# LTLA/batchelor

Measured on AMD Instinct MI355X. Metric: cells/sec corrected (reducedMNN engine, 50 PCs), higher is better.
Workload: dtype fp16 MFMA candidate pass (f32 accumulate) + FP64 exact re-rank; 1 GPU; config3: 8 synthetic Gaussian batches x 100000 cells x 50 PCs, k=20, merge.order=1..8, inputs resident in HBM; parallelism=single GPU, exact_fallback_queries=1050

## Files before the change

batchelor_amd/_lib.py:

```python
from __future__ import annotations

import ctypes
import os

import numpy as np

_HERE = os.path.dirname(os.path.abspath(__file__))
LIB_PATH = os.environ.get("BMX_LIB") or os.path.join(_HERE, "libbatchelor_mi355x.so")

c_i32p = ctypes.POINTER(ctypes.c_int32)
c_i64p = ctypes.POINTER(ctypes.c_int64)
c_f64p = ctypes.POINTER(ctypes.c_double)

_lib = None


class BatchelorMI355XError(RuntimeError):
    def __init__(self, code, message):
        super().__init__(message)
        self.code = code


def lib():
    global _lib
    if _lib is None:
        if not os.path.exists(LIB_PATH):
            raise ImportError(
                f"{LIB_PATH} is missing: build it with `python -c 'import __graft_entry__ as g; g.build()'` "
                "(or `make -C batchelor_amd/csrc`). There is no CPU fallback for the MI355X hot path.")
        try:
            import torch
        except Exception:
            pass
        _lib = ctypes.CDLL(LIB_PATH, mode=ctypes.RTLD_GLOBAL)
        _lib.bmx_last_error.restype = ctypes.c_char_p
        _lib.bmx_device_count.restype = ctypes.c_int32
        _lib.bmx_last_knn_exact_fallbacks.restype = ctypes.c_int64
        _lib.bmx_free.argtypes = [ctypes.c_void_p]
        _lib.bmx_free.restype = None
    return _lib


def check(rc):
    if rc != 0:
        raise BatchelorMI355XError(rc, lib().bmx_last_error().decode("utf-8", "replace"))


def dev_set(name, value):
    check(lib().bmx_dev_set(name.encode(), ctypes.c_int32(int(value))))


def dev_get(name):
    v = ctypes.c_int64(0)
    check(lib().bmx_dev_get(name.encode(), ctypes.byref(v)))
    return int(v.value)


def dev_get_bytes(name, n):
    out = np.zeros(int(n), dtype=np.uint8)
    check(lib().bmx_dev_get_bytes(name.encode(), out.ctypes.data_as(ctypes.c_void_p), ctypes.c_int64(int(n))))
    return out


def device_count():
    return int(lib().bmx_device_count())


def require_gpu():
    if device_count() < 1:
        raise BatchelorMI355XError(-1, "no MI355X / HIP device visible: the batchelor_amd hot path has no CPU fallback")


def f64p(a):
    return a.ctypes.data_as(c_f64p)


def i32p(a):
    return a.ctypes.data_as(c_i32p)


def as_f(a):
    return np.asfortranarray(a, dtype=np.float64)


# ... 8 lines not shown
```

batchelor_amd/csrc/abi.hip:

```cpp
#include <algorithm>
#include <chrono>
#include <climits>
#include <cstddef>
#include <cmath>
#include <cstdlib>
#include <cstring>
#include <functional>
#include <limits>
#include <memory>
#include <thread>
#include <vector>

#include "bmx_common.hpp"
#include "bmx_ops.hpp"
#include "engine.hpp"
#include "host_xfer.hpp"
#include "mnn_correct.hpp"
#include "rccl_dyn.hpp"
#include "resident_batches.hpp"

struct bmx_engine {
    std::unique_ptr<bmx::Engine> impl;
};
struct bmx_mnn_result {
    int B = 0;
    bmx::MnnCorrectResult r;
};

namespace {

thread_local std::string g_last_error;
thread_local int64_t g_last_fallbacks = 0;
thread_local int g_force_exact = 0;
thread_local std::unique_ptr<bmx::Engine> g_prim;

bmx::Engine& prim(int d) {
    if (!g_prim) {
        int dev = 0;
        BMX_HIP(hipGetDevice(&dev));
        g_prim = std::make_unique<bmx::Engine>(dev);
    }
    g_prim->d_ = d;
    g_prim->knn_ws_.force_exact = g_force_exact;
    return *g_prim;
}

template <class T>
T* upload(bmx::DevBuf<T>& buf, const T* host, size_t n, hipStream_t s) {
    T* p = buf.reserve(std::max<size_t>(n, 1));
// ... 115 lines not shown
        }
    });
}

void bmx_trim_caches(void) {
    bmx::DevBlockCache::release_global();
    bmx::StreamPool::release_all();
}

int64_t bmx_last_knn_exact_fallbacks(void) { return g_last_fallbacks; }

void bmx_set_force_exact_knn(int32_t on) { g_force_exact = on; }

int32_t bmx_dev_set(const char* name, int32_t value) {
    if (!name) return BMX_ERR_ARG;
    bmx::DevKnobs& k = bmx::dev_knobs();
    const std::string n(name);
    if (n == "knn_tier") k.knn_tier = value;
    else if (n == "sample") k.sample = value;
    else if (n == "split_c") k.split_c = value;
    else if (n == "force_c") k.force_c = value;
    else if (n == "no_margin") k.no_margin = value;
    else if (n == "asv_fast") k.asv_fast = value;
    else if (n == "asv_cap") k.asv_cap = value;
    else if (n == "sample_split") k.sample_split = value;
    else if (n == "lk_seed") k.lk_seed = value;
    else if (n == "asv_modes") k.asv_modes = value;
    else if (n == "asv_sync") k.asv_sync = value;
    else if (n == "tau_replay") k.tau_replay = value;
    else if (n == "exchange_always") k.exchange_always = value;
    else if (n == "refine_wave") k.refine_wave = value;
    else if (n == "asv_wide") k.asv_wide = value;
    else if (n == "asv_chunk") k.asv_chunk = value;
    else if (n == "reset") k = bmx::DevKnobs();
    else {
        g_last_error = "bmx_dev_set: unknown knob '" + n + "'";
        return BMX_ERR_ARG;
    }
    return BMX_OK;
}

int32_t bmx_dev_get(const char* name, int64_t* value) {
    if (!name || !value) return BMX_ERR_ARG;
    return guarded([&] {
        const std::string n(name);
        unsigned long long t[8];
        if (n == "asv_literal_cells" || n == "asv_fallback_cells" || n == "asv_tiled_cells") {
            bmx::asv_tally_read(t, false);
            *value = (int64_t)t[n == "asv_literal_cells" ? 0 : (n == "asv_fallback_cells" ? 1 : 2)];
        } else if (n == "asv_ticks_stream" || n == "asv_ticks_wait" || n == "asv_ticks_cells") {
            bmx::asv_ticks_read(t);
            *value = (int64_t)t[n == "asv_ticks_stream" ? 0 : (n == "asv_ticks_wait" ? 1 : 2)];
        } else if (n == "asv_ticks_literal" || n == "asv_ticks_chains" || n == "asv_literal_addends" || n == "asv_chain_tiles") {
            bmx::asv_ticks_read(t);
            *value = (int64_t)t[n == "asv_ticks_literal" ? 4 : (n == "asv_ticks_chains" ? 5 : (n == "asv_literal_addends" ? 6 : 7))];
        } else if (n == "delta_gene_tile" || n == "delta_pair_chunk") {
            *value = n == "delta_gene_tile" ? bmx::DELTA_GENE_TILE : bmx::DELTA_PAIR_CHUNK;
        } else if (n == "pca_sparse_row_segment") {
            *value = bmx::PCA_SPARSE_ROW_SEGMENT;
        } else if (n == "asv_tally_reset") {
            bmx::asv_tally_read(t, true);
            *value = 0;
        } else {
            throw bmx::Error(BMX_ERR_ARG, "bmx_dev_get: unknown counter '" + n + "'");
        }
    });
}

int32_t bmx_dev_get_bytes(const char* name, void* dst, int64_t n) {
    if (!name || (n > 0 && !dst) || n < 0) return BMX_ERR_ARG;
    return guarded([&] {
        if (std::string(name) != "asv_modes") throw bmx::Error(BMX_ERR_ARG, std::string("bmx_dev_get_bytes: unknown array '") + name + "'");
// ... 719 lines not shown
```

batchelor_amd/csrc/bmx_common.hpp:

```cpp
#pragma once
#include <hip/hip_runtime.h>

#include <atomic>
#include <cstdint>
#include <cstdio>
#include <map>
#include <mutex>
#include <stdexcept>
#include <string>
#include <vector>

#include "../../include/batchelor_mi355x.h"

namespace bmx {

struct Error : std::runtime_error {
    int code;
    Error(int c, const std::string& m) : std::runtime_error(m), code(c) {}
};

#define BMX_HIP(expr)                                                                                   \
    do {                                                                                                \
        hipError_t e_ = (expr);                                                                         \
        if (e_ != hipSuccess)                                                                           \
            throw bmx::Error(BMX_ERR_HIP, std::string(#expr) + " failed: " + hipGetErrorString(e_));    \
    } while (0)

#define BMX_LAUNCH_CHECK() BMX_HIP(hipGetLastError())

struct WatchdogTimeout : Error {
    explicit WatchdogTimeout(const std::string& m) : Error(BMX_ERR_HIP, m) {}
};
void guarded_stream_sync(hipStream_t stream, double budget_s);

#ifndef BMX_KS1
#define BMX_KS1 32
#endif

struct DevKnobs {
    int knn_tier = 0;
    int sample = -1;
    int split_c = 0;
    int force_c = 0;
    int no_margin = 0;
    int asv_fast = 0;
    int asv_cap = -1;
    int asv_modes = 0;
    int asv_sync = 0;
    int tau_replay = 0;
    int lk_seed = 1;
    int sample_split = -1;
    int exchange_always = 0;
    int refine_wave = 0;
    int asv_wide = 0;
    int asv_chunk = 0;
};
DevKnobs& dev_knobs();
bool debug_prints();
bool debug_timings();

inline int cdiv(int64_t a, int64_t b) { return (int)((a + b - 1) / b); }
inline int64_t round_up(int64_t a, int64_t b) { return (a + b - 1) / b * b; }

struct DevBlockCache {
    struct Block {
        void* p;
        size_t bytes;
        int device;
    };
    std::vector<Block> blocks;
    bool leak = false;
    DevBlockCache() = default;
    DevBlockCache(const DevBlockCache&) = delete;
    DevBlockCache& operator=(const DevBlockCache&) = delete;
    struct GlobalPool {
        std::mutex mu;
        std::vector<Block> blocks;
        size_t total = 0;
    };
    static GlobalPool& global() {
        static GlobalPool* g = new GlobalPool();
        return *g;
    }
    ~DevBlockCache() {
        GlobalPool& g = global();
        if (!leak) {
            std::lock_guard<std::mutex> lk(g.mu);
            for (const Block& b : blocks) {
// ... 298 lines not shown
        return events[events_used++];
    }
    ~KnnWorkspace() {
        if (abandon) return;
        pinned_small_give(pin_);
        for (auto& e : events) {
            (void)hipEventDestroy(e.first);
            (void)hipEventDestroy(e.second);
        }
    }
};

struct Bf16Launch {
    const uint16_t* pq;
    const uint16_t* pr;
    int nqb, first_begin, range_len, nranges, r_limit, out_chunk0, out_nchunks;
    uint32_t* tau_g;
    int sample;
    int32_t* cand;
    float* cand_v;
    float* tau;
    int n_full = 0;
    const float* margin = nullptr;
    int k = 0;
    const uint32_t* tau_seed = nullptr;
};
int bf16_pick_ns(int d);
int bf16_ncons(int NS, int KS);
void bf16_prep(hipStream_t stream, const double* X, const int32_t* rows, int n, int n_pad, int d, int NS,
               const double* mean, int is_query, uint16_t* P, double* n2, unsigned long long* maxbits,
               unsigned long long* slots);
bool bf16_launch(hipStream_t stream, KnnWorkspace& ws, int NS, int KS, const Bf16Launch& L);
int f16_rows_per_slot(int NS, int KS);

void knn_device(hipStream_t stream, KnnWorkspace& ws, const double* X, const int32_t* ref_rows, int nr,
                const double* Q, const int32_t* q_rows, int nq, int d, int k, int32_t* idx_out, double* dist_out,
                int q_begin, int q_end, const float* seed_d2 = nullptr, const double* centre = nullptr,
                double* kth_out = nullptr);

}
```

batchelor_amd/csrc/knn.hip:

```cpp
#include "bmx_common.hpp"
#include "knn_select.hpp"

#include <algorithm>
#include <atomic>
#include <chrono>
#include <cmath>
#include <cstdio>
#include <cstdlib>
#include <thread>

namespace bmx {

int f16_pick_ns(int d, int KS);
void f16_prep_all(hipStream_t stream, const double* X, const int32_t* rrows, int nr, int nr_pad, const double* Q,
                  const int32_t* qrows, int nq, int nq_pad, int d, int NS, const double* mean, uint16_t* Pr, uint16_t* Pq,
                  double* rn2, double* qn2, unsigned long long* maxbits, unsigned long long* slots, int32_t* flagged0,
                  float* margin, const sel::PassEps& pe, const float* seed_d2, uint32_t* tau_seed, uint32_t* tau_init);
bool f16_launch(hipStream_t stream, KnnWorkspace& ws, int NS, int KS, const Bf16Launch& L);
void f16_sample_merge(hipStream_t stream, const float* lists, int nranges, int KS, int nq, int k, const float* margin,
                      uint32_t* tau_g);

namespace {

using namespace sel;

constexpr int MAX_CHUNKS = 8;

__global__ void colsum_partial(const double* __restrict__ X, const int32_t* __restrict__ rows, int n, int d,
                               int rows_per_block, int stride, double* __restrict__ partial) {
    __shared__ double sm[4][64];
    const int c0 = threadIdx.x & 63, rl = threadIdx.x >> 6;
    const int r0 = blockIdx.x * rows_per_block;
    const int r1 = min(n, r0 + rows_per_block);
    for (int cb = 0; cb < d; cb += 64) {
        const int c = cb + c0;
        double s = 0.0;
        if (c < d)
            for (int r = r0 + rl; r < r1; r += 4) {
                const int64_t rs = (int64_t)r * stride;
                const int64_t row = rows ? rows[rs] : rs;
                s += X[row * d + c];
            }
        sm[rl][c0] = s;
        __syncthreads();
        if (rl == 0 && c < d) partial[(int64_t)blockIdx.x * d + c] = (sm[0][c0] + sm[1][c0]) + (sm[2][c0] + sm[3][c0]);
        __syncthreads();
    }
}

__global__ void colsum_final(const double* __restrict__ partial, int nblocks, int d, double scale,
                             double* __restrict__ out) {
    const int c = blockIdx.x * blockDim.x + threadIdx.x;
    if (c >= d) return;
    double s = 0.0;
    for (int b = 0; b < nblocks; ++b) s += partial[(int64_t)b * d + c];
    out[c] = s * scale;
}


// ... 31 lines not shown
        const double t = a[c] - b[c];
        s += t * t;
    }
    return s;
}

__device__ __forceinline__ bool key_less(double da, int ia, double db, int ib) {
    return da < db || (da == db && ia < ib);
}

constexpr int REFINE_MAXM = MAX_CHUNKS * 48;

__global__ void seed_tau_kernel(const float* __restrict__ seed_d2, const double* __restrict__ qn2,
                                const unsigned long long* __restrict__ max_rn2_bits, int nq, int nq_pad, PassEps pe,
                                uint32_t* __restrict__ tau_g) {
    const int q = blockIdx.x * blockDim.x + threadIdx.x;
    if (q >= nq_pad) return;
    uint32_t o = f32_orderable(-__builtin_inff());
    if (q < nq) o = pass_seed_tau((double)seed_d2[q], qn2[q], __longlong_as_double((long long)*max_rn2_bits), pe);
    tau_g[q] = q < nq ? min(tau_g[q], o) : o;
}

template <int REFINE_NC>
__global__ __launch_bounds__(256) void knn_refine(const double* __restrict__ X, const int32_t* __restrict__ ref_rows,
                                                  const double* __restrict__ Q, const int32_t* __restrict__ q_rows,
                                                  int nq, int d, int k, int KS, int nchunks, double eps_k, double eps_qr,
                                                  double eps_split, double eps_den, int scaled,
                                                  const int32_t* __restrict__ cand, const float* __restrict__ cand_v,
                                                  const float* __restrict__ tau, const double* __restrict__ qn2,
                                                  const unsigned long long* __restrict__ max_rn2_bits,
                                                  const float* __restrict__ seed_d2, int32_t* __restrict__ idx_out,
                                                  double* __restrict__ dist_out, int32_t* __restrict__ flagged,
                                                  double* __restrict__ flag_bound,
                                                  unsigned long long* __restrict__ zero_slots, int q0,
                                                  double* __restrict__ kth_out, int sq = 0) {
    __shared__ __attribute__((aligned(16))) double sd[4][REFINE_MAXM];
    __shared__ int si[4][REFINE_MAXM];
    const int lane = threadIdx.x & 63, w = threadIdx.x >> 6;
    if (zero_slots && blockIdx.x == 0 && threadIdx.x < 64) zero_slots[(size_t)threadIdx.x * 16] = 0ull;
    const int q = q0 + blockIdx.x * 4 + w;
    if (q >= nq) return;
    const int Mall = nchunks * KS;
    const double* qv = Q + (int64_t)(q_rows ? q_rows[q] : q) * d;
    const double max_rn2 = __longlong_as_double((long long)*max_rn2_bits);
    const double s = scaled ? pass_scale(max_rn2) : 1.0;
    const double s2inv = 1.0 / (s * s);
    const double eps = pass_eps(sqrt(qn2[q]), sqrt(max_rn2), s, eps_k, eps_qr, eps_split, eps_den);
    int M = 0;
    unsigned long long* sk = reinterpret_cast<unsigned long long*>(&sd[w][0]);
    for (int m0 = 0; m0 < Mall; m0 += 64) {
        const int m = m0 + lane;
        const int id = m < Mall ? cand[(int64_t)q * Mall + m] : -1;
        const unsigned long long mask = __builtin_amdgcn_ballot_w64(id >= 0);
        const int pos = M + __builtin_popcountll(mask & ((1ull << lane) - 1ull));
        if (id >= 0) {
            si[w][pos] = id;
            if (cand_v) sk[pos] = ((unsigned long long)f32_orderable(cand_v[(int64_t)q * Mall + m]) << 32) | (uint32_t)id;
        }
        M += __builtin_popcountll(mask);
    }
    __builtin_amdgcn_fence(__ATOMIC_ACQ_REL, "wavefront");
    float tmerge = __builtin_inff();
    if (cand_v && M > k) {
        constexpr int NU = (REFINE_MAXM + 63) / 64;
        int rk[NU], ids[NU];
        float vs[NU];
        float vk = __builtin_inff();
#pragma unroll
        for (int uu = 0; uu < NU; ++uu) {
            const int m = lane + 64 * uu;
            rk[uu] = 0x7FFFFFFF;
            ids[uu] = 0;
            vs[uu] = 0.f;
            if (m < M) {
                const unsigned long long km = sk[m];
                const float vm = orderable_f32((uint32_t)(km >> 32));
                int rank = 0;
                int f = 0;
                for (; f + 2 <= M; f += 2) {
                    typedef unsigned long long u64x2 __attribute__((ext_vector_type(2)));
                    const u64x2 kf = *reinterpret_cast<const u64x2*>(sk + f);
                    rank += (kf[0] < km ? 1 : 0) + (kf[1] < km ? 1 : 0);
                }
                if (f < M) rank += sk[f] < km ? 1 : 0;
                rk[uu] = rank;
                ids[uu] = (int)(uint32_t)km;
                vs[uu] = vm;
                if (rank == k - 1) vk = vm;
                if (rank == KS) tmerge = vm;
            }
// ... 55 lines not shown
                        const uint32_t lo = (uint32_t)__builtin_amdgcn_update_dpp(0, (int)(uint32_t)bits, 0x93, 0xF, 0xF, false);
                        const uint32_t hi = (uint32_t)__builtin_amdgcn_update_dpp(0, (int)(uint32_t)(bits >> 32), 0x93, 0xF, 0xF, false);
                        const double prev = __longlong_as_double((long long)(((unsigned long long)hi << 32) | lo));
                        double run = prev + y[c][0];
                        run += y[c][1];
                        if (p == ph && 4 * c + ph < np) acc = run;
                    }
                }
            }
            if (p == p_last && m < M) sd[w][m] = acc;
        }
    } else {
        for (int m = lane; m < M; m += 64) {
            const int id = si[w][m];
            sd[w][m] = exact_d2(qv, X + (int64_t)(ref_rows ? ref_rows[id] : id) * d, d);
        }
    }
    __builtin_amdgcn_fence(__ATOMIC_ACQ_REL, "wavefront");
    const double seed = seed_d2 ? (double)seed_d2[q] : __builtin_inf();
    double kth = M >= k ? 0.0 : seed;
    for (int m = M + lane; m < k; m += 64) idx_out[(int64_t)q * k + m] = seed_d2 ? -1 : 0;
    for (int m = lane; m < M; m += 64) {
        const double dm = sd[w][m];
        const int im = si[w][m];
        int rank = 0;
        for (int f = 0; f < M; ++f) rank += key_less(sd[w][f], si[w][f], dm, im) ? 1 : 0;
        if (rank < k) {
            idx_out[(int64_t)q * k + rank] = im;
            if (dist_out) dist_out[(int64_t)q * k + rank] = sq ? dm : sqrt(dm);
        }
        if (rank == k - 1) kth = dm;
    }
    float tmin = tmerge;
    for (int c = lane; c < nchunks; c += 64) tmin = fminf(tmin, tau[(int64_t)q * nchunks + c]);
    for (int o = 32; o > 0; o >>= 1) {
        tmin = fminf(tmin, __shfl_xor(tmin, o));
        kth = fmax(kth, __shfl_xor(kth, o));
    }
    const double kth_full = kth;
    kth = fmin(kth, seed);
    if (lane == 0) {
        const bool proven = kth < (double)tmin * s2inv + qn2[q] - eps;
        if (!proven) {
            const int pos = atomicAdd(&flagged[0], 1);
            flagged[1 + pos] = q;
            flag_bound[pos] = kth;
        }
        if (kth_out) kth_out[q] = (proven && M >= k) ? sqrt(kth_full) : __builtin_inf();
    }
}

template <int REFINE_NC>
__global__ __launch_bounds__(256) void knn_refine_half(const double* __restrict__ X, const int32_t* __restrict__ ref_rows,
                                                       const double* __restrict__ Q, const int32_t* __restrict__ q_rows,
                                                       int nq, int d, int k, int nchunks, double eps_k, double eps_qr,
                                                       double eps_split, double eps_den, int scaled,
                                                       const int32_t* __restrict__ cand, const float* __restrict__ cand_v,
                                                       const float* __restrict__ tau, const double* __restrict__ qn2,
                                                       const unsigned long long* __restrict__ max_rn2_bits,
                                                       const float* __restrict__ seed_d2, int32_t* __restrict__ idx_out,
                                                       double* __restrict__ dist_out, int32_t* __restrict__ flagged,
                                                       double* __restrict__ flag_bound,
                                                       unsigned long long* __restrict__ zero_slots,
                                                       double* __restrict__ kth_out, int sq = 0) {
    constexpr int KS = 32;
    __shared__ __attribute__((aligned(16))) double sd[8][KS];
    __shared__ int si[8][KS];
// ... 578 lines not shown

__global__ void tau_record_kernel(const float* __restrict__ tau, int nchunks, int nq, uint32_t* __restrict__ rec) {
    const int q = blockIdx.x * blockDim.x + threadIdx.x;
    if (q >= nq) return;
    float t = __builtin_inff();
    for (int c = 0; c < nchunks; ++c) t = fminf(t, tau[(int64_t)q * nchunks + c]);
    rec[q] = f32_orderable(t);
}
__global__ void tau_apply_kernel(const uint32_t* __restrict__ rec, int nq, uint32_t* __restrict__ tau_g) {
    const int q = blockIdx.x * blockDim.x + threadIdx.x;
    if (q < nq) tau_g[q] = min(tau_g[q], rec[q]);
}

#ifndef BMX_SEEDED_SAMPLE
#define BMX_SEEDED_SAMPLE 4096
#endif
struct Tier {
    int id;
    int NS, KS;
};

int candidate_tiers(int d, int k, int nr, Tier out[2]) {
    const int only = dev_knobs().knn_tier;
    int n = 0;
    if (k > 36) return 0;
    const int KS1 = k <= 20 ? BMX_KS1 : 48, KS2 = k <= 20 ? 24 : 40;
    const int ns1 = f16_pick_ns(d, KS1);
    if (ns1 && nr > 2 * KS1 && (only == 0 || only == 1)) out[n++] = Tier{1, ns1, KS1};
    const int ns2 = bf16_pick_ns(d);
    if (ns2 && !(KS2 == 40 && ns2 > 16) && nr > 2 * KS2 && (only == 0 || only == 2)) out[n++] = Tier{2, ns2, KS2};
    return n;
}

void candidate_pass(hipStream_t stream, KnnWorkspace& ws, const Tier& T, const double* X, const int32_t* ref_rows, int nr,
                    const double* Qs, const int32_t* qrs, int nq, int d, int k, int32_t* io, double* dout,
                    int32_t* flagged, double* flag_bound, const float* seed_d2, const double* centre, double* kth_out) {
    const int NS = T.NS, KS = T.KS;
    ws.last_variant = T.id == 1 ? 3 : 2;
    const int unit = T.id == 1 ? 256 : 32 * bf16_ncons(NS, KS);
    const int nq_pad = (int)round_up(nq, unit);
    const int nqb = nq_pad / unit;

    const bool no_margin_knob = dev_knobs().no_margin != 0;
    int S_auto = nr >= 32768 ? 4096 : 0;
    if (T.id == 1 && nr >= 4096) S_auto = std::max(1024, std::min(nr / 4, NS <= 4 ? 24576 : 12288));
    if (seed_d2 && T.id == 1) S_auto = std::min(S_auto, BMX_SEEDED_SAMPLE);
    int S = (int)round_up(dev_knobs().sample >= 0 ? dev_knobs().sample : S_auto, T.id == 1 ? f16_rows_per_slot(NS, KS) : 64);
    int CS = 1;
    if (T.id == 1 && S > 0 && nqb < 128 && dev_knobs().sample_split != 0 && !no_margin_knob) {
        const int rs = f16_rows_per_slot(NS, KS);
        CS = std::max(1, std::min({256 / std::max(nqb, 1), 8, S / (8 * rs)}));
        if (dev_knobs().sample_split > 0) CS = std::max(1, std::min({dev_knobs().sample_split, S / rs, 512 / KS}));
    }
    int C = 1, n_full = 0;
    {
        const int a = nqb / 256, b = nqb % 256;
        n_full = a * 256;
        if (b > 0) {
            double best = 1e30;
            for (int c = 1; c <= MAX_CHUNKS - 1; ++c) {
                if (c > 1 && nr / c < 2048) break;
                const double tailc = std::ceil((double)b * c / 256.0) / c * (1.0 + 0.105 * std::log((double)c));
                if (tailc < best - 1e-9) {
                    best = tailc;
                    C = c;
                }
            }
        }
    }
    if (dev_knobs().split_c > 0) C = std::max(1, dev_knobs().split_c);
    if (dev_knobs().force_c > 0) {
        C = std::max(1, std::min(MAX_CHUNKS - 1, dev_knobs().force_c));
        n_full = 0;
    }
    const int rmul = T.id == 1 ? f16_rows_per_slot(NS, KS) : 32;
    const int chunk_len = (int)round_up(cdiv(nr, C), rmul);
    C = std::max(1, cdiv(nr, chunk_len));
    const int nr_pad = chunk_len * C;
    const int nchunks = C;
    S = std::min(S, nr_pad / rmul * rmul);
    if (debug_prints())
        fprintf(stderr, "[bmx] knn tier %d: nq=%d nr=%d d=%d NS=%d KS=%d S=%d C=%d chunk=%d full-range blocks=%d of %d\n", T.id,
                nq, nr, d, NS, KS, S, C, chunk_len, C > 1 ? n_full : nqb, nqb);

    const int KPw = 8 * NS;
    float* pq = ws.pq.reserve((size_t)nq_pad * KPw);
    float* pr = ws.pr.reserve((size_t)(nr_pad + 256) * KPw);
    double* qn2 = ws.qn2.reserve(nq_pad);
    double* rn2 = ws.rn2.reserve(nr_pad);
    double* mean = ws.mean.reserve((size_t)d + 2);
    unsigned long long* maxbits = reinterpret_cast<unsigned long long*>(mean + d);
    int32_t* cand = ws.cand.reserve((size_t)nq_pad * nchunks * KS);
    float* cand_v = ws.cand_v.reserve((size_t)nq_pad * nchunks * KS);
    float* tau = ws.tau.reserve((size_t)nq_pad * nchunks);
    uint32_t* tau_g = ws.tau_g.reserve(nq_pad);
    unsigned long long* slots = ws.maxslots.reserve(64 * 16);

    if (!centre) {
        const int cstride = std::max(1, nr / 16384);
        const int ncs = cdiv(nr, cstride);
        const int rpb = 256;
        const int nb = cdiv(ncs, rpb);
        double* red = ws.red.reserve((size_t)nb * d);
        hipLaunchKernelGGL(colsum_partial, dim3(nb), dim3(256), 0, stream, X, ref_rows, ncs, d, rpb, cstride, red);
        BMX_LAUNCH_CHECK();
        hipLaunchKernelGGL(colsum_final, dim3(cdiv(d, 64)), dim3(64), 0, stream, red, nb, d, 1.0 / ncs, mean);
        BMX_LAUNCH_CHECK();
        centre = mean;
    }
    PassEps pe;
    if (T.id == 1) {
        pe.eps_k = 16.0 * NS;
        pe.eps_qr = 2.0;
        pe.eps_split = 2.0 * (0.0009765625 + 2.384185791015625e-07);
        pe.eps_den = 6.103515625e-05 * (std::sqrt((double)d) + 3.0);
        pe.scaled = 1;
    } else {
        pe.eps_k = 16.0 * NS;
        pe.eps_qr = 6.0;
        pe.eps_split = 1.5 * 3.03 * 2.0 * 1.52587890625e-05;
        pe.eps_den = 0.0;
        pe.scaled = 0;
    }
    const double eps_k = pe.eps_k, eps_qr = pe.eps_qr, eps_split = pe.eps_split, eps_den = pe.eps_den;
    Bf16Launch L{reinterpret_cast<const uint16_t*>(pq), reinterpret_cast<const uint16_t*>(pr), nqb, 0, S, 1, S, 0, nchunks,
                 tau_g, 1, cand, cand_v, tau};
    const bool no_margin = dev_knobs().no_margin != 0;
// ... 19 lines not shown
        if (S > 0) {
            float* lists = nullptr;
            if (CS > 1) {
                const int rs = f16_rows_per_slot(NS, KS);
                L.range_len = (int)round_up(cdiv(S, CS), rs);
                L.nranges = cdiv(S, L.range_len);
                if (L.nranges > 1 && margin) {
                    lists = ws.samp_lists.reserve((size_t)nq_pad * L.nranges * KS);
                    L.cand_v = lists;
                }
            }
            ok = go(L);
            if (lists) f16_sample_merge(stream, lists, L.nranges, KS, nq, k, margin, tau_g);
            L.cand_v = cand_v;
        }
    } else {
        ws.slots_clean = false;
        BMX_HIP(hipMemsetAsync(maxbits, 0, sizeof(unsigned long long), stream));
        bf16_prep(stream, X, ref_rows, nr, nr_pad, d, NS, centre, 0, reinterpret_cast<uint16_t*>(pr), rn2, maxbits, slots);
        bf16_prep(stream, Qs, qrs, nq, nq_pad, d, NS, centre, 1, reinterpret_cast<uint16_t*>(pq), qn2, maxbits, slots);
        if (S == 0) {
            hipLaunchKernelGGL(fill_u32, dim3(cdiv(nq_pad, 256)), dim3(256), 0, stream, tau_g, nq_pad, 0xFF800000u);
            BMX_LAUNCH_CHECK();
        }
        if (S > 0) ok = go(L);
        if (seed_d2) {
            hipLaunchKernelGGL(seed_tau_kernel, dim3(cdiv(nq_pad, 256)), dim3(256), 0, stream, seed_d2, qn2, maxbits, nq, nq_pad,
                               pe, tau_g);
            BMX_LAUNCH_CHECK();
        }
        BMX_HIP(hipMemsetAsync(flagged, 0, sizeof(int32_t), stream));
    }
    L.first_begin = 0;
    L.range_len = chunk_len;
    L.nranges = C;
    L.n_full = C > 1 ? n_full : 0;
    L.r_limit = nr_pad;
    L.sample = 0;
    const int replay = T.id == 1 ? dev_knobs().tau_replay : 0;
    if (replay == 2 && ws.replay_idx < ws.tau_rec.size() && ws.tau_rec[ws.replay_idx].cap >= (size_t)nq_pad) {
        hipLaunchKernelGGL(tau_apply_kernel, dim3(cdiv(nq_pad, 256)), dim3(256), 0, stream,
                           (const uint32_t*)ws.tau_rec[ws.replay_idx].p, nq_pad, tau_g);
        BMX_LAUNCH_CHECK();
    }
    ok = ok && go(L);
    if (replay == 1) {
        if (ws.tau_rec.size() <= ws.replay_idx) ws.tau_rec.resize(ws.replay_idx + 1);
        hipLaunchKernelGGL(tau_record_kernel, dim3(cdiv(nq_pad, 256)), dim3(256), 0, stream, (const float*)tau, nchunks, nq_pad,
                           ws.tau_rec[ws.replay_idx].reserve((size_t)nq_pad));
        BMX_LAUNCH_CHECK();
    }
    if (replay) ++ws.replay_idx;
    if (!ok) throw Error(BMX_ERR_ARG, "kNN: unsupported padded dimension");
    {
        const int need = (d & 1) ? 0 : cdiv(d, 8);
        const int unit_q = T.id == 1 ? 256 : 32 * bf16_ncons(NS, KS);
        const int nq_half = KS == 32 && !dev_knobs().refine_wave ? (C > 1 ? std::min(nq, n_full * unit_q) : nq) : 0;
        const int sq = ws.dist_squared ? 1 : 0;
#define BMX_REFINE(NC)                                                                                                              \
    do {                                                                                                                            \
        if (nq_half > 0)                                                                                                            \
            hipLaunchKernelGGL(knn_refine_half<NC>, dim3(cdiv(nq_half, 8)), dim3(256), 0, stream, X, ref_rows, Qs, qrs, nq_half, d, k, \
                               nchunks, eps_k, eps_qr, eps_split, eps_den, T.id == 1 ? 1 : 0, cand, cand_v, tau, qn2, maxbits,       \
                               seed_d2, io, dout, flagged, flag_bound, zero_slots, kth_out, sq);                                    \
        if (nq > nq_half)                                                                                                           \
            hipLaunchKernelGGL(knn_refine<NC>, dim3(cdiv(nq - nq_half, 4)), dim3(256), 0, stream, X, ref_rows, Qs, qrs, nq, d, k, KS,  \
                               nchunks, eps_k, eps_qr, eps_split, eps_den, T.id == 1 ? 1 : 0, cand, cand_v, tau, qn2, maxbits,       \
                               seed_d2, io, dout, flagged, flag_bound, nq_half > 0 ? nullptr : zero_slots, nq_half, kth_out, sq);   \
    } while (0)
        if (need == 0 || need > 16) BMX_REFINE(0);
        else if (need <= 2) BMX_REFINE(2);
        else if (need <= 4) BMX_REFINE(4);
        else if (need <= 7) BMX_REFINE(7);
        else if (need <= 10) BMX_REFINE(10);
        else if (need <= 13) BMX_REFINE(13);
        else BMX_REFINE(16);
#undef BMX_REFINE
    }
    BMX_LAUNCH_CHECK();
    if (zero_slots) ws.slots_clean = true;
    if (debug_prints()) {
        std::vector<int32_t> hc((size_t)nq * nchunks * KS);
        BMX_HIP(hipMemcpyAsync(hc.data(), cand, hc.size() * sizeof(int32_t), hipMemcpyDeviceToHost, stream));
        ws.sync(stream);
        size_t valid = 0;
        for (int32_t v : hc) valid += v >= 0;
        fprintf(stderr, "[bmx] candidates per query after the top-k pass: %.1f (of %d slots)\n", (double)valid / nq,
                nchunks * KS);
    }
}

__global__ void publish_word(const int32_t* __restrict__ dev, int32_t* host, int seq) {
    if (threadIdx.x != 0 || blockIdx.x != 0) return;
    const int32_t v = *dev;
    __hip_atomic_store(&host[0], v, __ATOMIC_RELAXED, __HIP_MEMORY_SCOPE_SYSTEM);
    __hip_atomic_store(&host[1], seq, __ATOMIC_RELEASE, __HIP_MEMORY_SCOPE_SYSTEM);
}

int read_count(hipStream_t stream, KnnWorkspace& ws, const int32_t* dev) {
    int32_t* h = reinterpret_cast<int32_t*>(ws.pinned_words());
    if (ws.read_seq == 0) h[1] = 0;
    const int seq = ++ws.read_seq;
    hipLaunchKernelGGL(publish_word, dim3(1), dim3(64), 0, stream, dev, h, seq);
    BMX_LAUNCH_CHECK();
    const double budget = ws.wd_budget_s;
    const auto t0 = std::chrono::steady_clock::now();
    volatile int32_t* vp = h;
    unsigned spins = 0;
    while (vp[1] != seq) {
        if ((++spins & 0x3FFu) == 0) {
            const double el = std::chrono::duration<double>(std::chrono::steady_clock::now() - t0).count();
            if (budget > 0.0 && el > budget)
                throw WatchdogTimeout("watchdog: the GPU work queued on the engine's stream did not finish in time; the engine is "
                                      "dead (restart the process)");
            if (el > 0.5) {
                const hipError_t e = hipStreamQuery(stream);
                (void)hipGetLastError();
                if (e != hipSuccess && e != hipErrorNotReady)
                    throw Error(BMX_ERR_HIP, std::string("the search's stream failed: ") + hipGetErrorString(e));
                std::this_thread::sleep_for(std::chrono::microseconds(200));
            }
// ... 640 lines not shown
```

include/batchelor_mi355x.h:

```cpp
#ifndef BATCHELOR_MI355X_H
#define BATCHELOR_MI355X_H

#include <stdint.h>

#ifdef __cplusplus
extern "C" {
#endif

#define BMX_OK 0
#define BMX_ERR_HIP (-1)
#define BMX_ERR_DIM_GENES (-2)
#define BMX_ERR_DIM_CELLS (-3)
#define BMX_ERR_SUBSET (-4)
#define BMX_ERR_INDEX_LEN (-5)
#define BMX_ERR_ARG (-6)
#define BMX_ERR_TREE (-7)
#define BMX_ERR_NO_PAIRS (-8)
#define BMX_ERR_EXCHANGE (-9)

const char* bmx_last_error(void);
int32_t bmx_device_count(void);
void bmx_free(void* p);
int32_t bmx_set_device(int32_t device);
void bmx_trim_caches(void);


int32_t bmx_find_mutual_nns(const int32_t* left, int32_t nL, int32_t k2, const int32_t* right, int32_t nR, int32_t k1,
                            int32_t** out_left, int32_t** out_right, int64_t* npairs);

int32_t bmx_smooth_gaussian_kernel(const double* averaged, int32_t g, int32_t U, const int32_t* index,
                                   int32_t index_len, const double* mat, int32_t gd, int32_t n, double sigma2,
                                   double* out);

int32_t bmx_adjust_shift_variance(const double* data1, int32_t g1, int32_t n1, const double* data2, int32_t g2,
                                  int32_t n2, const double* vect, int32_t vrow, int32_t vcol, double sigma2,
                                  const int32_t* restrict1, int32_t nr1, const int32_t* restrict2, int32_t nr2,
                                  double* out);

int32_t bmx_adjust_shift_variance_form(int32_t n2, int32_t nr1, int32_t nr2);


int32_t bmx_query_knn(const double* X, int32_t nx, const double* query, int32_t nq, int32_t d, int32_t k,
                      int32_t* index, double* distance);

int32_t bmx_find_mutual_nn(const double* data1, int32_t n1, const double* data2, int32_t n2, int32_t d, int32_t k1,
                           int32_t k2, int32_t** first, int32_t** second, int64_t* npairs);

int64_t bmx_last_knn_exact_fallbacks(void);
void bmx_set_force_exact_knn(int32_t on);
int32_t bmx_dev_set(const char* name, int32_t value);
int32_t bmx_dev_get(const char* name, int64_t* value);
int32_t bmx_dev_get_bytes(const char* name, void* dst, int64_t n);
double bmx_last_native_kernel_ms(void);
int32_t bmx_dev_host_copy(void* dst, const void* src, int64_t bytes);

typedef struct bmx_engine bmx_engine_t;

typedef struct {
    int32_t struct_size;
    int32_t k;
    double prop_k;
    double ndist;
    double min_batch_skip;
    int32_t auto_merge;
    int32_t var_adj;
    double sigma;
} bmx_params_t;

typedef int32_t (*bmx_allgather_fn)(void* ctx, void* buf, int64_t bytes_per_rank);

int32_t bmx_engine_create(int32_t device, bmx_engine_t** out);
void bmx_engine_destroy(bmx_engine_t* e);
int32_t bmx_engine_set_shard(bmx_engine_t* e, int32_t rank, int32_t world, bmx_allgather_fn fn, void* ctx);
int32_t bmx_rccl_load(const char* librccl_path);
int32_t bmx_rccl_unique_id(void* id_out, int32_t bytes);
int32_t bmx_engine_init_rccl(bmx_engine_t* e, int32_t rank, int32_t world, const void* unique_id, int32_t bytes);
int32_t bmx_engine_exchange_stats(bmx_engine_t* e, int64_t* calls, int64_t* bytes);
int32_t bmx_engine_upload(bmx_engine_t* e, int32_t nbatches, int32_t d, const double* const* data,
                          const int32_t* nrows, const int32_t* const* restrict_idx, const int32_t* n_restrict);
int32_t bmx_engine_run(bmx_engine_t* e, const bmx_params_t* params, const int32_t* tree, int32_t tree_len);
int32_t bmx_engine_download(bmx_engine_t* e, double* corrected, int32_t* batch, int32_t* merge_left,
                            int32_t* merge_right, double* batch_size, int32_t* skipped, double* lost_var);
int32_t bmx_engine_pairs(bmx_engine_t* e, int32_t merge, int32_t** left, int32_t** right, int64_t* npairs);
// ... 183 lines not shown
```

Baseline: 9.238 million cells/s.

## Plan kNN candidate tail as two query groups with different reference splits

Replaces the single chunk-count choice for the tail of query blocks with a cost-model planner that may split the tail into two groups, each using its own number of reference ranges, and launches a second candidate pass plus a separate refine launch for the second group. The wave count now comes from the device's CU count instead of a hard-coded 256. The aim is to cut idle compute units in the last wave of the candidate pass. In exchange it adds an extra launch, different candidate-buffer offsets and a planner whose constants are heuristic.

New measurement: 9.173 million cells/s. Within noise of the previous version (-0.7%).

```diff
diff --git a/batchelor_amd/_lib.py b/batchelor_amd/_lib.py
--- a/batchelor_amd/_lib.py
+++ b/batchelor_amd/_lib.py
@@ -50,6 +50,17 @@
     check(lib().bmx_dev_set(name.encode(), ctypes.c_int32(int(value))))
 
 
+def knn_plan(nqb, nr, d=50, k=20, slots=0):
+    out = np.zeros(12, dtype=np.int32)
+    cost = np.zeros(2, dtype=np.float64)
+    check(lib().bmx_knn_plan(ctypes.c_int32(int(nqb)), ctypes.c_int32(int(nr)), ctypes.c_int32(int(d)), ctypes.c_int32(int(k)),
+                             ctypes.c_int32(int(slots)), i32p(out), f64p(cost)))
+    groups = [dict(first=int(out[2 + 4 * g]), blocks=int(out[3 + 4 * g]), ranges=int(out[4 + 4 * g]),
+                   range_len=int(out[5 + 4 * g])) for g in range(int(out[1]))]
+    return dict(n_full=int(out[0]), groups=groups, rows_per_slot=int(out[10]), max_chunks=int(out[11]),
+                cost=float(cost[0]), cost_single=float(cost[1]))
+
+
 def dev_get(name):
     v = ctypes.c_int64(0)
     check(lib().bmx_dev_get(name.encode(), ctypes.byref(v)))
diff --git a/batchelor_amd/csrc/abi.hip b/batchelor_amd/csrc/abi.hip
--- a/batchelor_amd/csrc/abi.hip
+++ b/batchelor_amd/csrc/abi.hip
@@ -15,6 +15,7 @@
 #include "bmx_ops.hpp"
 #include "engine.hpp"
 #include "host_xfer.hpp"
+#include "knn_plan.hpp"
 #include "mnn_correct.hpp"
 #include "rccl_dyn.hpp"
 #include "resident_batches.hpp"
@@ -196,12 +197,48 @@
     else if (n == "refine_wave") k.refine_wave = value;
     else if (n == "asv_wide") k.asv_wide = value;
     else if (n == "asv_chunk") k.asv_chunk = value;
+    else if (n == "plan_slots") k.plan_slots = value;
+    else if (n == "plan_groups") k.plan_groups = value;
+    else if (n == "plan_c1") k.plan_c1 = value;
+    else if (n == "plan_b2") k.plan_b2 = value;
+    else if (n == "plan_c2") k.plan_c2 = value;
+    else if (n == "plan_only_b") k.plan_only_b = value;
     else if (n == "reset") k = bmx::DevKnobs();
     else {
         g_last_error = "bmx_dev_set: unknown knob '" + n + "'";
         return BMX_ERR_ARG;
     }
     return BMX_OK;
+}
+
+int32_t bmx_knn_plan(int32_t nqb, int32_t nr, int32_t d, int32_t k, int32_t slots, int32_t* out, double* cost) {
+    if (!out || !cost) return BMX_ERR_ARG;
+    return guarded([&] {
+        const bmx::DevKnobs& kn = bmx::dev_knobs();
+        if (slots <= 0) slots = kn.plan_slots;
+        if (slots <= 0) throw bmx::Error(BMX_ERR_ARG, "bmx_knn_plan: a slot count (argument or the knob plan_slots): no device is asked");
+        if (nqb < 0 || nr < 1 || d < 1 || k < 1 || k > 36) throw bmx::Error(BMX_ERR_ARG, "bmx_knn_plan: shape outside the candidate tiers");
+        const int KS = k <= 20 ? BMX_KS1 : 48;
+        const int NS = bmx::f16_pick_ns(d, KS);
+        if (!NS) throw bmx::Error(BMX_ERR_ARG, "bmx_knn_plan: the fp16 tier does not take rows of that length");
+        const int rmul = bmx::f16_rows_per_slot(NS, KS);
+        const bool forced = kn.plan_only_b <= 0 || nqb % slots == kn.plan_only_b;
+        const bmx::KnnPlan P = bmx::plan_knn(nqb, nr, rmul, bmx::KNN_MIN_RANGE, bmx::KNN_MAX_CHUNKS, slots, kn.plan_groups == 1 ? 1 : 0,
+                                             forced ? bmx::KnnPlanForce{kn.plan_c1, kn.plan_b2, kn.plan_c2} : bmx::KnnPlanForce());
+        out[0] = P.n_full;
+        out[1] = P.ngroups;
+        for (int g = 0; g < 2; ++g) {
+            const bool on = g < P.ngroups;
+            out[2 + 4 * g] = on ? P.g[g].first : 0;
+            out[3 + 4 * g] = on ? P.g[g].blocks : 0;
+            out[4 + 4 * g] = on ? P.g[g].ranges : 0;
+            out[5 + 4 * g] = on ? P.g[g].range_len : 0;
+        }
+        out[10] = rmul;
+        out[11] = bmx::KNN_MAX_CHUNKS;
+        cost[0] = P.cost;
+        cost[1] = P.cost_single;
+    });
 }
 
 int32_t bmx_dev_get(const char* name, int64_t* value) {
diff --git a/batchelor_amd/csrc/bmx_common.hpp b/batchelor_amd/csrc/bmx_common.hpp
--- a/batchelor_amd/csrc/bmx_common.hpp
+++ b/batchelor_amd/csrc/bmx_common.hpp
@@ -54,6 +54,12 @@
     int refine_wave = 0;
     int asv_wide = 0;
     int asv_chunk = 0;
+    int plan_slots = 0;
+    int plan_groups = 0;
+    int plan_c1 = 0;
+    int plan_b2 = 0;
+    int plan_c2 = 0;
+    int plan_only_b = 0;
 };
 DevKnobs& dev_knobs();
 bool debug_prints();
@@ -418,6 +424,9 @@
                unsigned long long* slots);
 bool bf16_launch(hipStream_t stream, KnnWorkspace& ws, int NS, int KS, const Bf16Launch& L);
 int f16_rows_per_slot(int NS, int KS);
+int f16_pick_ns(int d, int KS);
+constexpr int KNN_MAX_CHUNKS = 8;
+constexpr int KNN_MIN_RANGE = 2048;
 
 void knn_device(hipStream_t stream, KnnWorkspace& ws, const double* X, const int32_t* ref_rows, int nr,
                 const double* Q, const int32_t* q_rows, int nq, int d, int k, int32_t* idx_out, double* dist_out,
diff --git a/batchelor_amd/csrc/knn.hip b/batchelor_amd/csrc/knn.hip
--- a/batchelor_amd/csrc/knn.hip
+++ b/batchelor_amd/csrc/knn.hip
@@ -1,4 +1,5 @@
 #include "bmx_common.hpp"
+#include "knn_plan.hpp"
 #include "knn_select.hpp"
 
 #include <algorithm>
@@ -11,7 +12,6 @@
 
 namespace bmx {
 
-int f16_pick_ns(int d, int KS);
 void f16_prep_all(hipStream_t stream, const double* X, const int32_t* rrows, int nr, int nr_pad, const double* Q,
                   const int32_t* qrows, int nq, int nq_pad, int d, int NS, const double* mean, uint16_t* Pr, uint16_t* Pq,
                   double* rn2, double* qn2, unsigned long long* maxbits, unsigned long long* slots, int32_t* flagged0,
@@ -24,7 +24,7 @@
 
 using namespace sel;
 
-constexpr int MAX_CHUNKS = 8;
+constexpr int MAX_CHUNKS = KNN_MAX_CHUNKS;
 
 __global__ void colsum_partial(const double* __restrict__ X, const int32_t* __restrict__ rows, int n, int d,
                                int rows_per_block, int stride, double* __restrict__ partial) {
@@ -122,15 +122,16 @@
                                                   const float* __restrict__ seed_d2, int32_t* __restrict__ idx_out,
                                                   double* __restrict__ dist_out, int32_t* __restrict__ flagged,
                                                   double* __restrict__ flag_bound,
-                                                  unsigned long long* __restrict__ zero_slots, int q0,
+                                                  unsigned long long* __restrict__ zero_slots, int q0, int q1,
                                                   double* __restrict__ kth_out, int sq = 0) {
     __shared__ __attribute__((aligned(16))) double sd[4][REFINE_MAXM];
     __shared__ int si[4][REFINE_MAXM];
     const int lane = threadIdx.x & 63, w = threadIdx.x >> 6;
     if (zero_slots && blockIdx.x == 0 && threadIdx.x < 64) zero_slots[(size_t)threadIdx.x * 16] = 0ull;
     const int q = q0 + blockIdx.x * 4 + w;
-    if (q >= nq) return;
+    if (q >= q1) return;
     const int Mall = nchunks * KS;
+    const int64_t ql = q - q0;
     const double* qv = Q + (int64_t)(q_rows ? q_rows[q] : q) * d;
     const double max_rn2 = __longlong_as_double((long long)*max_rn2_bits);
     const double s = scaled ? pass_scale(max_rn2) : 1.0;
@@ -140,12 +141,12 @@
     unsigned long long* sk = reinterpret_cast<unsigned long long*>(&sd[w][0]);
     for (int m0 = 0; m0 < Mall; m0 += 64) {
         const int m = m0 + lane;
-        const int id = m < Mall ? cand[(int64_t)q * Mall + m] : -1;
+        const int id = m < Mall ? cand[ql * Mall + m] : -1;
         const unsigned long long mask = __builtin_amdgcn_ballot_w64(id >= 0);
         const int pos = M + __builtin_popcountll(mask & ((1ull << lane) - 1ull));
         if (id >= 0) {
             si[w][pos] = id;
-            if (cand_v) sk[pos] = ((unsigned long long)f32_orderable(cand_v[(int64_t)q * Mall + m]) << 32) | (uint32_t)id;
+            if (cand_v) sk[pos] = ((unsigned long long)f32_orderable(cand_v[ql * Mall + m]) << 32) | (uint32_t)id;
         }
         M += __builtin_popcountll(mask);
     }
@@ -267,7 +268,7 @@
         if (rank == k - 1) kth = dm;
     }
     float tmin = tmerge;
-    for (int c = lane; c < nchunks; c += 64) tmin = fminf(tmin, tau[(int64_t)q * nchunks + c]);
+    for (int c = lane; c < nchunks; c += 64) tmin = fminf(tmin, tau[ql * nchunks + c]);
     for (int o = 32; o > 0; o >>= 1) {
         tmin = fminf(tmin, __shfl_xor(tmin, o));
         kth = fmax(kth, __shfl_xor(kth, o));
@@ -912,6 +913,21 @@
     return n;
 }
 
+int plan_slots() {
+    if (dev_knobs().plan_slots > 0) return dev_knobs().plan_slots;
+    static std::atomic<int> cus[64];
+    int dev = 0;
+    BMX_HIP(hipGetDevice(&dev));
+    const int slot = dev >= 0 && dev < 64 ? dev : 0;
+    int n = cus[slot].load(std::memory_order_relaxed);
+    if (n <= 0 || slot != dev) {
+        BMX_HIP(hipDeviceGetAttribute(&n, hipDeviceAttributeMultiprocessorCount, dev));
+        n = std::max(1, n);
+        if (slot == dev) cus[slot].store(n, std::memory_order_relaxed);
+    }
+    return n;
+}
+
 void candidate_pass(hipStream_t stream, KnnWorkspace& ws, const Tier& T, const double* X, const int32_t* ref_rows, int nr,
                     const double* Qs, const int32_t* qrs, int nq, int d, int k, int32_t* io, double* dout,
                     int32_t* flagged, double* flag_bound, const float* seed_d2, const double* centre, double* kth_out) {
@@ -932,36 +948,49 @@
         CS = std::max(1, std::min({256 / std::max(nqb, 1), 8, S / (8 * rs)}));
         if (dev_knobs().sample_split > 0) CS = std::max(1, std::min({dev_knobs().sample_split, S / rs, 512 / KS}));
     }
-    int C = 1, n_full = 0;
-    {
-        const int a = nqb / 256, b = nqb % 256;
-        n_full = a * 256;
-        if (b > 0) {
-            double best = 1e30;
-            for (int c = 1; c <= MAX_CHUNKS - 1; ++c) {
-                if (c > 1 && nr / c < 2048) break;
-                const double tailc = std::ceil((double)b * c / 256.0) / c * (1.0 + 0.105 * std::log((double)c));
-                if (tailc < best - 1e-9) {
-                    best = tailc;
-                    C = c;
-                }
-            }
-        }
-    }
-    if (dev_knobs().split_c > 0) C = std::max(1, dev_knobs().split_c);
-    if (dev_knobs().force_c > 0) {
-        C = std::max(1, std::min(MAX_CHUNKS - 1, dev_knobs().force_c));
-        n_full = 0;
-    }
     const int rmul = T.id == 1 ? f16_rows_per_slot(NS, KS) : 32;
-    const int chunk_len = (int)round_up(cdiv(nr, C), rmul);
-    C = std::max(1, cdiv(nr, chunk_len));
-    const int nr_pad = chunk_len * C;
+    const DevKnobs& kn = dev_knobs();
+    const int wg_slots = plan_slots();
+    const bool grouped = T.id == 1 && kn.split_c <= 0 && kn.force_c <= 0 && kn.tau_replay == 0;
+    KnnPlanForce force;
+    if (grouped && (kn.plan_only_b <= 0 || nqb % wg_slots == kn.plan_only_b)) force = KnnPlanForce{kn.plan_c1, kn.plan_b2, kn.plan_c2};
+    KnnPlan P = plan_knn(nqb, nr, rmul, KNN_MIN_RANGE, MAX_CHUNKS, wg_slots,
+                         grouped && (kn.plan_groups ? kn.plan_groups : KNN_PLAN_DEFAULT_GROUPS) != 1 ? 0 : 1, force);
+    if (kn.split_c > 0 || kn.force_c > 0) {
+        int C = kn.split_c > 0 ? std::max(1, kn.split_c) : 1;
+        if (kn.force_c > 0) {
+            C = std::max(1, std::min(MAX_CHUNKS - 1, kn.force_c));
+            P.n_full = 0;
+        }
+        P.ngroups = 1;
+        P.g[0].first = P.n_full;
+        P.g[0].blocks = nqb - P.n_full;
+        P.g[0].range_len = (int)round_up(cdiv(nr, C), rmul);
+        P.g[0].ranges = std::max(1, cdiv(nr, P.g[0].range_len));
+    }
+    if (P.ngroups == 0) {
+        P.g[0].first = P.n_full;
+        P.g[0].blocks = 0;
+        P.g[0].ranges = 1;
+        P.g[0].range_len = (int)round_up(nr, rmul);
+    }
+    int C = P.g[0].ranges;
+    const int chunk_len = P.g[0].range_len;
+    const int n_full = C > 1 ? P.n_full : 0;
+    const int nq2b = P.ngroups == 2 ? P.g[1].blocks : 0;
+    const int nq1b = nqb - nq2b;
+    const int C2 = nq2b ? P.g[1].ranges : 0, chunk_len2 = nq2b ? P.g[1].range_len : 0;
+    const int q2_first = nq1b * unit;
+    const int nr_pad1 = chunk_len * C, nr_pad2 = chunk_len2 * C2;
+    const int nr_pad = std::max(nr_pad1, nr_pad2);
     const int nchunks = C;
     S = std::min(S, nr_pad / rmul * rmul);
     if (debug_prints())
-        fprintf(stderr, "[bmx] knn tier %d: nq=%d nr=%d d=%d NS=%d KS=%d S=%d C=%d chunk=%d full-range blocks=%d of %d\n", T.id,
-                nq, nr, d, NS, KS, S, C, chunk_len, C > 1 ? n_full : nqb, nqb);
+        fprintf(stderr,
+                "[bmx] knn tier %d: nq=%d nr=%d d=%d NS=%d KS=%d S=%d C=%d chunk=%d full-range blocks=%d of %d | plan for %d slots: "
+                "%d whole, %d x %d ranges of %d, %d x %d ranges of %d (model %.0f, single split %.0f tiles)\n",
+                T.id, nq, nr, d, NS, KS, S, C, chunk_len, C > 1 ? n_full : nq1b, nqb, wg_slots, C > 1 ? n_full : nq1b,
+                C > 1 ? nq1b - n_full : 0, C, chunk_len, nq2b, C2, chunk_len2, P.cost, P.cost_single);
 
     const int KPw = 8 * NS;
     float* pq = ws.pq.reserve((size_t)nq_pad * KPw);
@@ -970,9 +999,13 @@
     double* rn2 = ws.rn2.reserve(nr_pad);
     double* mean = ws.mean.reserve((size_t)d + 2);
     unsigned long long* maxbits = reinterpret_cast<unsigned long long*>(mean + d);
-    int32_t* cand = ws.cand.reserve((size_t)nq_pad * nchunks * KS);
-    float* cand_v = ws.cand_v.reserve((size_t)nq_pad * nchunks * KS);
-    float* tau = ws.tau.reserve((size_t)nq_pad * nchunks);
+    const size_t lists1 = (size_t)nq1b * unit * nchunks, lists2 = (size_t)nq2b * unit * C2;
+    int32_t* cand = ws.cand.reserve((lists1 + lists2) * KS);
+    float* cand_v = ws.cand_v.reserve((lists1 + lists2) * KS);
+    float* tau = ws.tau.reserve(lists1 + lists2);
+    int32_t* cand2 = cand + lists1 * KS;
+    float* cand2_v = cand_v + lists1 * KS;
+    float* tau2 = tau + lists1;
     uint32_t* tau_g = ws.tau_g.reserve(nq_pad);
     unsigned long long* slots = ws.maxslots.reserve(64 * 16);
 
@@ -1058,10 +1091,11 @@
         BMX_HIP(hipMemsetAsync(flagged, 0, sizeof(int32_t), stream));
     }
     L.first_begin = 0;
+    L.nqb = nq1b;
     L.range_len = chunk_len;
     L.nranges = C;
-    L.n_full = C > 1 ? n_full : 0;
-    L.r_limit = nr_pad;
+    L.n_full = n_full;
+    L.r_limit = nr_pad1;
     L.sample = 0;
     const int replay = T.id == 1 ? dev_knobs().tau_replay : 0;
     if (replay == 2 && ws.replay_idx < ws.tau_rec.size() && ws.tau_rec[ws.replay_idx].cap >= (size_t)nq_pad) {
@@ -1070,6 +1104,23 @@
         BMX_LAUNCH_CHECK();
     }
     ok = ok && go(L);
+    if (nq2b) {
+        Bf16Launch L2 = L;
+        L2.pq = L.pq + (size_t)q2_first * KPw * 2;
+        L2.nqb = nq2b;
+        L2.n_full = 0;
+        L2.range_len = chunk_len2;
+        L2.nranges = C2;
+        L2.r_limit = nr_pad2;
+        L2.out_nchunks = C2;
+        L2.tau_g = tau_g + q2_first;
+        if (L.margin) L2.margin = L.margin + q2_first;
+        if (L.tau_seed) L2.tau_seed = L.tau_seed + q2_first;
+        L2.cand = cand2;
+        L2.cand_v = cand2_v;
+        L2.tau = tau2;
+        ok = ok && go(L2);
+    }
     if (replay == 1) {
         if (ws.tau_rec.size() <= ws.replay_idx) ws.tau_rec.resize(ws.replay_idx + 1);
         hipLaunchKernelGGL(tau_record_kernel, dim3(cdiv(nq_pad, 256)), dim3(256), 0, stream, (const float*)tau, nchunks, nq_pad,
@@ -1080,8 +1131,8 @@
     if (!ok) throw Error(BMX_ERR_ARG, "kNN: unsupported padded dimension");
     {
         const int need = (d & 1) ? 0 : cdiv(d, 8);
-        const int unit_q = T.id == 1 ? 256 : 32 * bf16_ncons(NS, KS);
-        const int nq_half = KS == 32 && !dev_knobs().refine_wave ? (C > 1 ? std::min(nq, n_full * unit_q) : nq) : 0;
+        const int nq1 = std::min(nq, q2_first);
+        const int nq_half = KS == 32 && !dev_knobs().refine_wave ? (C > 1 ? std::min(nq1, n_full * unit) : nq1) : 0;
         const int sq = ws.dist_squared ? 1 : 0;
 #define BMX_REFINE(NC)                                                                                                              \
     do {                                                                                                                            \
@@ -1089,10 +1140,15 @@
             hipLaunchKernelGGL(knn_refine_half<NC>, dim3(cdiv(nq_half, 8)), dim3(256), 0, stream, X, ref_rows, Qs, qrs, nq_half, d, k, \
                                nchunks, eps_k, eps_qr, eps_split, eps_den, T.id == 1 ? 1 : 0, cand, cand_v, tau, qn2, maxbits,       \
                                seed_d2, io, dout, flagged, flag_bound, zero_slots, kth_out, sq);                                    \
-        if (nq > nq_half)                                                                                                           \
-            hipLaunchKernelGGL(knn_refine<NC>, dim3(cdiv(nq - nq_half, 4)), dim3(256), 0, stream, X, ref_rows, Qs, qrs, nq, d, k, KS,  \
-                               nchunks, eps_k, eps_qr, eps_split, eps_den, T.id == 1 ? 1 : 0, cand, cand_v, tau, qn2, maxbits,       \
-                               seed_d2, io, dout, flagged, flag_bound, nq_half > 0 ? nullptr : zero_slots, nq_half, kth_out, sq);   \
+        if (nq1 > nq_half)                                                                                                          \
+            hipLaunchKernelGGL(knn_refine<NC>, dim3(cdiv(nq1 - nq_half, 4)), dim3(256), 0, stream, X, ref_rows, Qs, qrs, nq, d, k, KS, \
+                               nchunks, eps_k, eps_qr, eps_split, eps_den, T.id == 1 ? 1 : 0, cand + (size_t)nq_half * nchunks * KS, \
+                               cand_v + (size_t)nq_half * nchunks * KS, tau + (size_t)nq_half * nchunks, qn2, maxbits, seed_d2, io,  \
+                               dout, flagged, flag_bound, nq_half > 0 ? nullptr : zero_slots, nq_half, nq1, kth_out, sq);           \
+        if (nq > nq1)                                                                                                               \
+            hipLaunchKernelGGL(knn_refine<NC>, dim3(cdiv(nq - nq1, 4)), dim3(256), 0, stream, X, ref_rows, Qs, qrs, nq, d, k, KS,    \
+                               C2, eps_k, eps_qr, eps_split, eps_den, T.id == 1 ? 1 : 0, cand2, cand2_v, tau2, qn2, maxbits,        \
+                               seed_d2, io, dout, flagged, flag_bound, nq1 > 0 ? nullptr : zero_slots, nq1, nq, kth_out, sq);       \
     } while (0)
         if (need == 0 || need > 16) BMX_REFINE(0);
         else if (need <= 2) BMX_REFINE(2);
@@ -1106,13 +1162,13 @@
     BMX_LAUNCH_CHECK();
     if (zero_slots) ws.slots_clean = true;
     if (debug_prints()) {
-        std::vector<int32_t> hc((size_t)nq * nchunks * KS);
+        std::vector<int32_t> hc((lists1 + lists2) * KS);
         BMX_HIP(hipMemcpyAsync(hc.data(), cand, hc.size() * sizeof(int32_t), hipMemcpyDeviceToHost, stream));
         ws.sync(stream);
         size_t valid = 0;
         for (int32_t v : hc) valid += v >= 0;
-        fprintf(stderr, "[bmx] candidates per query after the top-k pass: %.1f (of %d slots)\n", (double)valid / nq,
-                nchunks * KS);
+        fprintf(stderr, "[bmx] candidates per query after the top-k pass: %.1f (of %d slots, group 2: %d)\n", (double)valid / nq,
+                nchunks * KS, C2 * KS);
     }
 }
 
diff --git a/batchelor_amd/csrc/knn_plan.hpp b/batchelor_amd/csrc/knn_plan.hpp
--- /dev/null
+++ b/batchelor_amd/csrc/knn_plan.hpp
@@ -0,0 +1,150 @@
+#pragma once
+#include <algorithm>
+#include <cmath>
+#include <cstdint>
+
+namespace bmx {
+
+constexpr double KNN_PLAN_SPLIT_LN = 0.105;
+constexpr double KNN_PLAN_ITEM_TILES = 40.0;
+constexpr double KNN_PLAN_LAUNCH_TILES = 40.0;
+constexpr int KNN_PLAN_DEFAULT_GROUPS = 2;
+
+struct KnnPlanGroup {
+    int first = 0;
+    int blocks = 0;
+    int ranges = 1;
+    int range_len = 0;
+};
+
+struct KnnPlan {
+    int n_full = 0;
+    int ngroups = 0;
+    KnnPlanGroup g[2];
+    double cost = 0.0;
+    double cost_single = 0.0;
+};
+
+struct KnnPlanForce {
+    int c1 = 0, b2 = 0, c2 = 0;
+};
+
+namespace knn_plan_detail {
+inline int cdiv_i(int64_t a, int64_t b) { return (int)((a + b - 1) / b); }
+inline int round_up_i(int64_t a, int64_t b) { return (int)((a + b - 1) / b * b); }
+
+inline void ranges_for(int nr, int c, int rmul, int& ranges, int& range_len) {
+    range_len = round_up_i(cdiv_i(nr, std::max(1, c)), rmul);
+    ranges = std::max(1, cdiv_i(nr, range_len));
+}
+inline double item_cost(int range_len, int ranges) {
+    return (double)(range_len / 32) * (1.0 + KNN_PLAN_SPLIT_LN * std::log((double)ranges)) + KNN_PLAN_ITEM_TILES;
+}
+inline double group_cost(int blocks, int ranges, int range_len, int slots) {
+    return blocks > 0 ? (double)cdiv_i((int64_t)blocks * ranges, slots) * item_cost(range_len, ranges) : 0.0;
+}
+}
+
+inline KnnPlan plan_knn(int nqb, int nr, int rmul, int min_range, int max_chunks, int slots, int groups = 0,
+                        KnnPlanForce force = KnnPlanForce()) {
+    using namespace knn_plan_detail;
+    KnnPlan P;
+    slots = std::max(1, slots);
+    rmul = std::max(32, rmul);
+    nqb = std::max(0, nqb);
+    nr = std::max(1, nr);
+    const int cmax = std::max(1, max_chunks - 1);
+    const int a = nqb / slots, b = nqb % slots;
+    P.n_full = a * slots;
+    int len1, one;
+    ranges_for(nr, 1, rmul, one, len1);
+    const double full = (double)a * item_cost(len1, 1);
+    if (b == 0) {
+        P.cost = P.cost_single = full;
+        return P;
+    }
+    int C = 1;
+    {
+        double best = 1e30;
+        for (int c = 1; c <= cmax; ++c) {
+            if (c > 1 && nr / c < min_range) break;
+            const double tailc = std::ceil((double)b * c / (double)slots) / c * (1.0 + 0.105 * std::log((double)c));
+            if (tailc < best - 1e-9) {
+                best = tailc;
+                C = c;
+            }
+        }
+    }
+    KnnPlanGroup s;
+    s.first = P.n_full;
+    s.blocks = b;
+    ranges_for(nr, C, rmul, s.ranges, s.range_len);
+    P.ngroups = 1;
+    P.g[0] = s;
+    P.cost = P.cost_single = full + group_cost(b, s.ranges, s.range_len, slots);
+
+    auto two = [&](int b1, int c1, int c2, KnnPlan& out) {
+        out = P;
+        out.ngroups = 2;
+        out.g[0].first = P.n_full;
+        out.g[0].blocks = b1;
+        ranges_for(nr, c1, rmul, out.g[0].ranges, out.g[0].range_len);
+        out.g[1].first = P.n_full + b1;
+        out.g[1].blocks = b - b1;
+        ranges_for(nr, c2, rmul, out.g[1].ranges, out.g[1].range_len);
+        out.cost = full + group_cost(b1, out.g[0].ranges, out.g[0].range_len, slots) +
+                   group_cost(b - b1, out.g[1].ranges, out.g[1].range_len, slots) + KNN_PLAN_LAUNCH_TILES;
+    };
+    if (force.c1 > 0 || force.b2 > 0 || force.c2 > 0) {
+        const int climit = std::min(cmax, std::max(1, nr / rmul));
+        const int c1 = std::max(1, std::min(climit, force.c1 > 0 ? force.c1 : s.ranges));
+        const int c2 = std::max(1, std::min(climit, force.c2 > 0 ? force.c2 : c1));
+        const int b2 = std::max(0, std::min(b - 1, force.b2));
+        if (b2 == 0) {
+            ranges_for(nr, c1, rmul, P.g[0].ranges, P.g[0].range_len);
+            P.cost = full + group_cost(b, P.g[0].ranges, P.g[0].range_len, slots);
+        } else {
+            KnnPlan F;
+            two(b - b2, c1, c2, F);
+            P = F;
+        }
+        return P;
+    }
+    if (groups == 1 || b < 2) return P;
+    constexpr int CTAB = 64;
+    double item[CTAB];
+    int ncs = 0;
+    for (int c = 1; c <= cmax && c < CTAB; ++c) {
+        if (c > 1 && nr / c < min_range) break;
+        int rg, len;
+        ranges_for(nr, c, rmul, rg, len);
+        item[c] = item_cost(len, rg);
+        ncs = c;
+    }
+    double best_cost = P.cost;
+    int best_b1 = 0, best_c1 = 0, best_c2 = 0;
+    for (int c1 = 1; c1 <= ncs; ++c1) {
+        const int rounds = cdiv_i((int64_t)b * c1, slots);
+        for (int m = 1; m <= rounds; ++m) {
+            const int b1 = (int)std::min<int64_t>(b - 1, (int64_t)m * slots / c1);
+            if (b1 < 1) continue;
+            const double head = full + KNN_PLAN_LAUNCH_TILES + (double)cdiv_i((int64_t)b1 * c1, slots) * item[c1];
+            for (int c2 = 1; c2 <= ncs; ++c2) {
+                if (c2 == c1) continue;
+                const double cost = head + (double)cdiv_i((int64_t)(b - b1) * c2, slots) * item[c2];
+                if (cost < best_cost * (1.0 - 1e-9)) {
+                    best_cost = cost;
+                    best_b1 = b1;
+                    best_c1 = c1;
+                    best_c2 = c2;
+                }
+            }
+        }
+    }
+    if (best_b1 == 0) return P;
+    KnnPlan best;
+    two(best_b1, best_c1, best_c2, best);
+    return best;
+}
+
+}
diff --git a/include/batchelor_mi355x.h b/include/batchelor_mi355x.h
--- a/include/batchelor_mi355x.h
+++ b/include/batchelor_mi355x.h
@@ -49,6 +49,7 @@
 int64_t bmx_last_knn_exact_fallbacks(void);
 void bmx_set_force_exact_knn(int32_t on);
 int32_t bmx_dev_set(const char* name, int32_t value);
+int32_t bmx_knn_plan(int32_t nqb, int32_t nr, int32_t d, int32_t k, int32_t slots, int32_t* out, double* cost);
 int32_t bmx_dev_get(const char* name, int64_t* value);
 int32_t bmx_dev_get_bytes(const char* name, void* dst, int64_t n);
 double bmx_last_native_kernel_ms(void);
```
